# richhiey/YourMT3

Measured on AMD Instinct MI355X. Metric: audio-sec transcribed / wall-sec (RTF), higher is better.
Workload: dtype bf16; 1 GPU; BASELINE configs[1]: MT3 base (T5-small dims, 6+6 layers, d512, 8x64 heads, d_ff 2048, vocab 1536), 2.048 s / 16 kHz / 128-mel segments (256 encoder frames), greedy decode forced to 1024 tokens, seeded random weights; segments_per_gpu=64, global_batch=64, decode_len=1024, frames=256, parallelism=dp1 (segments sharded, token ids all-gathered over RCCL)

## Files before the change

yourmt3_amd/csrc/dec_chain.hip:

```cpp
#include <cstdlib>

#include "common.h"
#include "kernels.h"

namespace {

#include "dec_chain_body.h"

template <int MODE3, bool W2F>
__global__ __launch_bounds__(512) void dec_chain_kernel(const bf16_t* __restrict__ pW0, const bf16_t* __restrict__ pW1, const bf16_t* __restrict__ pW2,
                                                        const bf16_t* __restrict__ pW3, const bf16_t* __restrict__ pAttn, float* pH, int row0, int R,
                                                        ChainArgs c) {
    extern __shared__ __attribute__((aligned(16))) char smem[];
    chain_stages<MODE3, W2F>(pW0, pW1, pW2, pW3, pAttn, pH, row0, R, c, smem, blockIdx.x);
}

__global__ void chain_poison_kernel(const unsigned* sync, int32_t* tokens, float* scores, long long n) {
    if (sync[CHAIN_ABORT_WORD] == 0u) return;
    for (long long i = (long long)blockIdx.x * blockDim.x + threadIdx.x; i < n; i += (long long)gridDim.x * blockDim.x) {
        tokens[i] = INT32_MIN;
        if (scores) scores[i] = __builtin_nanf("");
    }
}

constexpr size_t CHAIN_LDS = (size_t)(8 * 16 * 16 + 16) * 4 + (size_t)8 * 2 * 16 * (2048 / 8 * 2 + 16);
constexpr size_t CHAIN_LDS_W2F = (size_t)(8 * 16 * 16 + 16) * 4 + (size_t)8 * 16 * (2048 / 8 * 2 + 16);
constexpr size_t CHAIN_LDS_NORM = (size_t)(8 * 16 * 32 + 16) * 4 + (size_t)8 * 3 * 16 * (512 / 8 * 2 + 16);
static_assert(CHAIN_LDS >= CHAIN_LDS_NORM && CHAIN_LDS_W2F >= CHAIN_LDS_NORM, "NORM stage LDS");
static_assert(CHAIN_LDS_W2F <= 80 * 1024, "two workgroups per CU");

}

int init_chain_kernels() {
    int rc = 0;
    rc |= hipFuncSetAttribute(reinterpret_cast<const void*>(dec_chain_kernel<DG_NORM_QKV_CACHE, false>), hipFuncAttributeMaxDynamicSharedMemorySize, (int)CHAIN_LDS) != hipSuccess;
    rc |= hipFuncSetAttribute(reinterpret_cast<const void*>(dec_chain_kernel<DG_NORM_LOGITS, false>), hipFuncAttributeMaxDynamicSharedMemorySize, (int)CHAIN_LDS) != hipSuccess;
    rc |= hipFuncSetAttribute(reinterpret_cast<const void*>(dec_chain_kernel<DG_NORM_QKV_CACHE, true>), hipFuncAttributeMaxDynamicSharedMemorySize, (int)CHAIN_LDS_W2F) != hipSuccess;
    rc |= hipFuncSetAttribute(reinterpret_cast<const void*>(dec_chain_kernel<DG_NORM_LOGITS, true>), hipFuncAttributeMaxDynamicSharedMemorySize, (int)CHAIN_LDS_W2F) != hipSuccess;
    return rc ? -2 : 0;
}

static bool chain_w2f() {
    static const bool v = [] { const char* e = getenv("YMT3_CHAIN_W2F"); return e && e[0] == '1'; }();
    return v;
}

bool dec_chain_fits(int n_cus) {
    int a = 0, b = 0;
    if (chain_w2f()) {
        if (hipOccupancyMaxActiveBlocksPerMultiprocessor(&a, dec_chain_kernel<DG_NORM_QKV_CACHE, true>, 512, CHAIN_LDS_W2F) != hipSuccess) return false;
        if (hipOccupancyMaxActiveBlocksPerMultiprocessor(&b, dec_chain_kernel<DG_NORM_LOGITS, true>, 512, CHAIN_LDS_W2F) != hipSuccess) return false;
    } else {
        if (hipOccupancyMaxActiveBlocksPerMultiprocessor(&a, dec_chain_kernel<DG_NORM_QKV_CACHE, false>, 512, CHAIN_LDS) != hipSuccess) return false;
        if (hipOccupancyMaxActiveBlocksPerMultiprocessor(&b, dec_chain_kernel<DG_NORM_LOGITS, false>, 512, CHAIN_LDS) != hipSuccess) return false;
    }
    return (long long)(a < b ? a : b) * n_cus >= 256;
}

int launch_dec_chain(const ChainArgs& c, hipStream_t stream) {
    if (c.R <= 0) return 0;
    if (c.R > 16 * CHAIN_TILES_MAX || c.d_ff != 2048 || c.N3 % 32 || c.N3 / 32 < 32 || c.N3 / 32 > 64 || !c.sync || (c.mode3 != DG_NORM_QKV_CACHE && c.mode3 != DG_NORM_LOGITS))
        return -1;
    const int n_mt = (c.R + 15) / 16;
    const int grid = n_mt <= 4 ? 256 : 64 * n_mt;
    if (chain_w2f()) {
        if (c.mode3 == DG_NORM_QKV_CACHE)
            dec_chain_kernel<DG_NORM_QKV_CACHE, true><<<grid, 512, CHAIN_LDS_W2F, stream>>>(c.w0, c.w1, c.w2, c.w3, c.attn, c.h, c.row0, c.R, c);
        else
            dec_chain_kernel<DG_NORM_LOGITS, true><<<grid, 512, CHAIN_LDS_W2F, stream>>>(c.w0, c.w1, c.w2, c.w3, c.attn, c.h, c.row0, c.R, c);
    } else if (c.mode3 == DG_NORM_QKV_CACHE)
        dec_chain_kernel<DG_NORM_QKV_CACHE, false><<<grid, 512, CHAIN_LDS, stream>>>(c.w0, c.w1, c.w2, c.w3, c.attn, c.h, c.row0, c.R, c);
    else
        dec_chain_kernel<DG_NORM_LOGITS, false><<<grid, 512, CHAIN_LDS, stream>>>(c.w0, c.w1, c.w2, c.w3, c.attn, c.h, c.row0, c.R, c);
    return 0;
}

int launch_chain_poison(const unsigned* sync, int32_t* tokens, float* scores, long long n, hipStream_t stream) {
    if (!sync || !tokens || n <= 0) return 0;
    chain_poison_kernel<<<64, 256, 0, stream>>>(sync, tokens, scores, n);
    return 0;
}
```

yourmt3_amd/csrc/dec_chain_body.h:

```cpp
#pragma once

#ifndef YMT3_TID
#define YMT3_TID threadIdx.x
#endif
#ifndef YMT3_POLL_PAUSE
#define YMT3_POLL_PAUSE do { } while (0)
#endif

typedef unsigned u32x4 __attribute__((ext_vector_type(4)));
constexpr int DKV = 64;
constexpr int AGENT = 16;
constexpr unsigned long long SPIN_LIMIT = 100000000ull;

#define CH_STAMP_IN(c) do { if ((c).stamp && YMT3_TID == 0) (c).stamp[2 * blockIdx.x] = wall_clock64(); } while (0)
#define CH_MARK(c, k) do { if ((c).stamp && YMT3_TID == 0) (c).stamp[512 + 8 * blockIdx.x + (k)] = wall_clock64(); } while (0)
#define CH_STAMP_OUT(c) do { if ((c).stamp && (YMT3_TID & 63) == 0) atomicMax((c).stamp + 2 * blockIdx.x + 1, (unsigned long long)wall_clock64()); } while (0)

__device__ __forceinline__ __amdgpu_buffer_rsrc_t raw_rsrc(const void* p) {
    return __builtin_amdgcn_make_buffer_rsrc(const_cast<void*>(p), 0, 0x7fffffff, 0x00020000);
}
__device__ __forceinline__ u32x4 ld16_agent(__amdgpu_buffer_rsrc_t r, int byte_off) { return __builtin_amdgcn_raw_buffer_load_b128(r, byte_off, 0, AGENT); }
__device__ __forceinline__ float ld_agent(const float* p) { return __hip_atomic_load(p, __ATOMIC_RELAXED, __HIP_MEMORY_SCOPE_AGENT); }
__device__ __forceinline__ void st_agent(float* p, float v) { __hip_atomic_store(p, v, __ATOMIC_RELAXED, __HIP_MEMORY_SCOPE_AGENT); }
__device__ __forceinline__ void st_agent(uint32_t* p, uint32_t v) { __hip_atomic_store(p, v, __ATOMIC_RELAXED, __HIP_MEMORY_SCOPE_AGENT); }
__device__ __forceinline__ void st2_agent(float* p, float2 v) {
    __hip_atomic_store(reinterpret_cast<unsigned long long*>(p), __builtin_bit_cast(unsigned long long, v), __ATOMIC_RELAXED, __HIP_MEMORY_SCOPE_AGENT);
}

template <int K, int NT>
struct Geo {
    static constexpr int KW = K / 8, KS = KW / 32, COLS = 16 * NT, PITCH = KW * 2 + 16, STRIP = 16 * PITCH;
    static constexpr int LPRW = KW * 2 / 16, RPIW = 64 / LPRW, NIA = 16 / RPIW, NIW = NIA * NT;
    static constexpr int LPRX = KW * 4 / 16, RPIX = 64 / LPRX, NIX = 16 / RPIX;
};

template <int K, int NT>
__device__ __forceinline__ void load_w(const bf16_t* W, int n0, u32x4 (&wv)[Geo<K, NT>::NIW]) {
    using G = Geo<K, NT>;
    const int lane = YMT3_TID & 63, wave = YMT3_TID >> 6;
#pragma unroll
    for (int i = 0; i < G::NIW; ++i)
        wv[i] = *reinterpret_cast<const u32x4*>(W + (size_t)(n0 + i * G::RPIW + lane / G::LPRW) * K + wave * G::KW + (lane % G::LPRW) * 8);
}

template <int K>
__device__ __forceinline__ void load_w_frag(const bf16_t* W, int n0, u32x4 (&wf)[Geo<K, 1>::KS]) {
    using G = Geo<K, 1>;
    const int lane = YMT3_TID & 63, wave = YMT3_TID >> 6, li = lane & 15, g = lane >> 4;
#pragma unroll
    for (int ks = 0; ks < G::KS; ++ks)
        wf[ks] = *reinterpret_cast<const u32x4*>(W + (size_t)(n0 + li) * K + wave * G::KW + ks * 32 + g * 8);
}

__device__ __forceinline__ unsigned* chain_counter(unsigned* sync, int boundary, int mt, int replica) {
    return sync + ((boundary * CHAIN_TILES_MAX + mt) * 8 + replica) * CHAIN_LINE;
}
__device__ __forceinline__ void chain_wait(unsigned* sync, int boundary, int mt, unsigned target, unsigned* host_abort, unsigned* abort_at = nullptr, int nsub = 1) {
    if (YMT3_TID < 64) {
        const int lane = YMT3_TID;
        const unsigned* cnt = chain_counter(sync, boundary, mt + 4 * (lane < nsub ? lane : 0), blockIdx.x & 7);
        const unsigned each = target / (unsigned)nsub;
        unsigned* abort_word = abort_at ? abort_at : sync + CHAIN_ABORT_WORD;
        unsigned long long t0 = 0;
        unsigned polls = 0;
        for (;;) {
            unsigned v = each;
            if (lane < nsub) v = __hip_atomic_load(cnt, __ATOMIC_RELAXED, __HIP_MEMORY_SCOPE_AGENT);
            if (__ballot(v < each) == 0ull) break;
            YMT3_POLL_PAUSE;
            if ((++polls & 63u) == 0u) {
                const unsigned long long now = wall_clock64();
                if (t0 == 0) t0 = now;
                if (__hip_atomic_load(abort_word, __ATOMIC_RELAXED, __HIP_MEMORY_SCOPE_AGENT) || now - t0 > SPIN_LIMIT) {
                    if (lane == 0) {
                        __hip_atomic_store(abort_word, 1u, __ATOMIC_RELAXED, __HIP_MEMORY_SCOPE_AGENT);
                        if (host_abort) __hip_atomic_store(host_abort, 1u, __ATOMIC_RELAXED, __HIP_MEMORY_SCOPE_SYSTEM);
                    }
                    break;
                }
            }
        }
    }
    __syncthreads();
}
__device__ __forceinline__ void counter_wait(const unsigned* cnt, unsigned target, unsigned* abort_word, unsigned* host_abort) {
    if (YMT3_TID == 0) {
        unsigned long long t0 = 0;
        unsigned polls = 0;
        while (__hip_atomic_load(cnt, __ATOMIC_RELAXED, __HIP_MEMORY_SCOPE_AGENT) < target) {
            YMT3_POLL_PAUSE;
            if ((++polls & 63u) == 0u) {
                const unsigned long long now = wall_clock64();
                if (t0 == 0) t0 = now;
                if (__hip_atomic_load(abort_word, __ATOMIC_RELAXED, __HIP_MEMORY_SCOPE_AGENT) || now - t0 > SPIN_LIMIT) {
                    __hip_atomic_store(abort_word, 1u, __ATOMIC_RELAXED, __HIP_MEMORY_SCOPE_AGENT);
                    if (host_abort) __hip_atomic_store(host_abort, 1u, __ATOMIC_RELAXED, __HIP_MEMORY_SCOPE_SYSTEM);
                    break;
                }
            }
        }
    }
    __syncthreads();
}
__device__ __forceinline__ void counter_signal(unsigned* cnt, int n, int stride) {
    asm volatile("s_waitcnt vmcnt(0)" ::: "memory");
    __syncthreads();
    if ((int)YMT3_TID < n) __hip_atomic_fetch_add(cnt + YMT3_TID * stride, 1u, __ATOMIC_RELAXED, __HIP_MEMORY_SCOPE_AGENT);
}
__device__ __forceinline__ void chain_signal(unsigned* sync, int boundary, int mt, int sub = 0) {
    asm volatile("s_waitcnt vmcnt(0)" ::: "memory");
    __syncthreads();
    if (YMT3_TID < 8) __hip_atomic_fetch_add(chain_counter(sync, boundary, mt + 4 * sub, YMT3_TID), 1u, __ATOMIC_RELAXED, __HIP_MEMORY_SCOPE_AGENT);
}

template <int K, int NT>
__device__ __forceinline__ float2 mfma_reduce(char* sA, char* sW, float* red) {
    using G = Geo<K, NT>;
    const int tid = YMT3_TID, lane = tid & 63, wave = tid >> 6, li = lane & 15, g = lane >> 4;
    f32x4 acc[NT];
#pragma unroll
    for (int c = 0; c < NT; ++c) acc[c] = (f32x4){0.f, 0.f, 0.f, 0.f};
#pragma unroll
    for (int ks = 0; ks < G::KS; ++ks) {
        const int off = li * G::PITCH + (ks * 32 + g * 8) * 2;
        const bf16x8 af = *reinterpret_cast<const bf16x8*>(sA + off);
#pragma unroll
        for (int c = 0; c < NT; ++c) {
            const bf16x8 wf = *reinterpret_cast<const bf16x8*>(sW + c * G::STRIP + off);
            acc[c] = __builtin_amdgcn_mfma_f32_16x16x32_bf16(wf, af, acc[c], 0, 0, 0);
        }
    }
#pragma unroll
    for (int c = 0; c < NT; ++c)
        *reinterpret_cast<float4*>(red + ((wave * 16 + li) * G::COLS + c * 16 + g * 4)) = make_float4(acc[c][0], acc[c][1], acc[c][2], acc[c][3]);
    __syncthreads();
    float2 s = make_float2(0.f, 0.f);
    if (tid < 16 * 8 * NT) {
        const int mr = tid / (8 * NT), nq = (tid % (8 * NT)) * 2;
        s = *reinterpret_cast<const float2*>(red + (mr * G::COLS + nq));
#pragma unroll
        for (int w = 1; w < 8; ++w) {
            const float2 t = *reinterpret_cast<const float2*>(red + ((w * 16 + mr) * G::COLS + nq));
            s.x += t.x; s.y += t.y;
        }
    }
    return s;
}

template <int K>
__device__ __forceinline__ float2 mfma_reduce_wfrag(char* sA, const u32x4 (&wfr)[Geo<K, 1>::KS], float* red) {
    using G = Geo<K, 1>;
    const int tid = YMT3_TID, lane = tid & 63, wave = tid >> 6, li = lane & 15, g = lane >> 4;
    f32x4 acc = (f32x4){0.f, 0.f, 0.f, 0.f};
#pragma unroll
    for (int ks = 0; ks < G::KS; ++ks) {
        const bf16x8 af = *reinterpret_cast<const bf16x8*>(sA + li * G::PITCH + (ks * 32 + g * 8) * 2);
        acc = __builtin_amdgcn_mfma_f32_16x16x32_bf16(__builtin_bit_cast(bf16x8, wfr[ks]), af, acc, 0, 0, 0);
    }
    *reinterpret_cast<float4*>(red + ((wave * 16 + li) * 16 + g * 4)) = make_float4(acc[0], acc[1], acc[2], acc[3]);
    __syncthreads();
    float2 s = make_float2(0.f, 0.f);
    if (tid < 16 * 8) {
        const int mr = tid / 8, nq = (tid % 8) * 2;
        s = *reinterpret_cast<const float2*>(red + (mr * 16 + nq));
#pragma unroll
        for (int w = 1; w < 8; ++w) {
            const float2 t = *reinterpret_cast<const float2*>(red + ((w * 16 + mr) * 16 + nq));
            s.x += t.x; s.y += t.y;
        }
    }
    return s;
}

__device__ __forceinline__ float2 resid_out(float2 hold, float2 s, float* pH, float* pSsq, int ssq_stride, int m, int n, int nt_idx, bool live) {
    float2 o = make_float2(0.f, 0.f);
    if (live) {
        o = make_float2(hold.x + s.x, hold.y + s.y);
        st2_agent(pH + (size_t)m * 512 + n, o);
    }
    float q = add_sep(mul_sep(o.x, o.x), mul_sep(o.y, o.y));
    q = sum8(q);
    if (live && (YMT3_TID & 7) == 0) st_agent(pSsq + (size_t)nt_idx * ssq_stride + m, q);
    return o;
}

__device__ __forceinline__ f32x4 norm_gain(const float* gain) {
    using G = Geo<512, 2>;
    return *reinterpret_cast<const f32x4*>(gain + (YMT3_TID >> 6) * G::KW + ((YMT3_TID & 63) % G::LPRX) * 4);
}
template <int NT>
__device__ __forceinline__ void norm_park(char* smem, u32x4 (&wv)[Geo<512, NT>::NIW]) {
    using G = Geo<512, NT>;
    const int lane = YMT3_TID & 63, wave = YMT3_TID >> 6;
    char* sW = smem + (8 * 16 * G::COLS + 16) * 4 + wave * (1 + NT) * G::STRIP + G::STRIP;
#pragma unroll
    for (int i = 0; i < G::NIW; ++i)
        *reinterpret_cast<u32x4*>(sW + (i * G::RPIW + lane / G::LPRW) * G::PITCH + (lane % G::LPRW) * 16) = wv[i];
}

template <int MODE, bool INL = false>
__device__ __forceinline__ void norm_tile(const ChainArgs& c, const float* pH, int row0, int R, const f32x4 gv, int N, int nt_idx, int mt_idx,
                                          int step, char* smem) {
    using G = Geo<512, 2>;
    constexpr int NT = 2;
    float* red = reinterpret_cast<float*>(smem);
    float* sscale = red + 8 * 16 * G::COLS;
    char* strips = smem + (8 * 16 * G::COLS + 16) * 4;
    const int tid = YMT3_TID, lane = tid & 63, wave = tid >> 6;
    const int n0 = nt_idx * G::COLS, m0 = row0 + mt_idx * 16, m_end = row0 + R;
    char* sA = strips + wave * (1 + NT) * G::STRIP;
    char* sW = sA + G::STRIP;
    const __amdgpu_buffer_rsrc_t rx = raw_rsrc(pH);
    f32x4 xv[G::NIX];
#pragma unroll
    for (int i = 0; i < G::NIX; ++i) {
        int mm = m0 + i * G::RPIX + lane / G::LPRX;
        mm = mm < m_end ? mm : m_end - 1;
        xv[i] = __builtin_bit_cast(f32x4, ld16_agent(rx, (mm * 512 + wave * G::KW + (lane % G::LPRX) * 4) * 4));
    }
    float ss = 0.f;
    if (tid < 16 * 8) {
        const int mm = m0 + (tid >> 3) < m_end ? m0 + (tid >> 3) : m_end - 1;
#pragma unroll
        for (int j = 0; j < 4; ++j) ss += ld_agent(c.ssq + (size_t)((tid & 7) * 4 + j) * c.ssq_stride + mm);
    }
    ss = sum8(ss);
    if (tid < 16 * 8 && (tid & 7) == 0) sscale[tid >> 3] = rsqrtf(ss / 512.f + c.eps);
    __syncthreads();
#pragma unroll
    for (int i = 0; i < G::NIX; ++i) {
        const int row = i * G::RPIX + lane / G::LPRX;
        const float sc = sscale[row];
        *reinterpret_cast<uint2*>(sA + row * G::PITCH + (lane % G::LPRX) * 8) =
            make_uint2(pack_bf16x2(xv[i][0] * sc * gv[0], xv[i][1] * sc * gv[1]), pack_bf16x2(xv[i][2] * sc * gv[2], xv[i][3] * sc * gv[3]));
    }
    float2 s = mfma_reduce<512, NT>(sA, sW, red);
    const bool epi = tid < 16 * 8 * NT;
    const int mr = tid / (8 * NT), nq = (tid % (8 * NT)) * 2;
    const int m = m0 + mr, n = n0 + nq;
    if (!(epi && m < m_end)) return;
    if constexpr (MODE == DG_NORM_LOGITS) {
        *reinterpret_cast<float2*>(c.logits + (size_t)m * N + n) = s;
    } else if constexpr (MODE == DG_NORM_BF16_RELU) {
        s.x = fmaxf(s.x, 0.f); s.y = fmaxf(s.y, 0.f);
        st_agent(reinterpret_cast<uint32_t*>(c.dff + (size_t)m * N + n), pack_bf16x2(s.x, s.y));
    } else {
        const uint32_t pk = pack_bf16x2(s.x, s.y);
        const int inner = c.H * DKV;
        if (n < inner) {
            if constexpr (INL) st_agent(reinterpret_cast<uint32_t*>(c.out_q + (size_t)m * inner + n), pk);
            else *reinterpret_cast<uint32_t*>(c.out_q + (size_t)m * inner + n) = pk;
        } else {
            const int nn = n - inner, kv = nn / inner, hh = (nn % inner) >> 6, dd = nn & 63;
            bf16_t* cache = kv ? c.vcache : c.kcache;
            if constexpr (INL) st_agent(reinterpret_cast<uint32_t*>(cache + (((size_t)m * c.H + hh) * c.L + step) * DKV + dd), pk);
            else *reinterpret_cast<uint32_t*>(cache + (((size_t)m * c.H + hh) * c.L + step) * DKV + dd) = pk;
        }
    }
}

struct ChainInLaunch {
    const unsigned* attn_done;
    unsigned attn_target;
    unsigned* qkv_done;
    unsigned long long* mark;
    int tiles_free;
};
template <int MODE3, bool W2F, bool INL = false>
__device__ __forceinline__ void chain_stages(const bf16_t* __restrict__ pW0, const bf16_t* __restrict__ pW1, const bf16_t* __restrict__ pW2,
                                             const bf16_t* __restrict__ pW3, const bf16_t* __restrict__ pAttn, float* pH, int row0, int R,
                                             const ChainArgs& c, char* smem, int t, const ChainInLaunch in = ChainInLaunch{}) {
    using G0 = Geo<512, 1>;
    using G1 = Geo<512, 2>;
    using G2 = Geo<2048, 1>;
    const int tid = YMT3_TID, lane = tid & 63, wave = tid >> 6;
    const int n_mt = (R + 15) / 16, m_end = row0 + R;
    const int nsub_all = c.nsub ? c.nsub : 0x444;
    const int nsub0 = n_mt <= 4 ? nsub_all & 15 : 1, nsub1 = n_mt <= 4 ? (nsub_all >> 4) & 15 : 1, nsub2 = n_mt <= 4 ? (nsub_all >> 8) & 15 : 1;
    const int mt = n_mt <= 4 ? (t >> 3) & 3 : t >> 6, nt = n_mt <= 4 ? (t >> 5) * 8 + (t & 7) : t & 63;
    const int n_nt3 = c.N3 / 32;
    const bool has0 = mt < n_mt && nt < 32, has1 = mt < n_mt, has3 = mt < n_mt && nt < n_nt3;
    const int nt0 = nt & 31, mt0 = mt, nt1 = nt, mt1 = mt, nt3 = nt < n_nt3 ? nt : nt - n_nt3, mt3 = mt;

    u32x4 w0[G0::NIW], av[G0::NIA];
    load_w<512, 1>(pW0, nt0 * 16, w0);
    const int m0 = row0 + mt0 * 16;
    const bool epi0 = tid < 16 * 8;
    const int mr0 = tid / 8, nq0 = (tid % 8) * 2;
    const int mE = m0 + mr0, nE = nt0 * 16 + nq0;
    const bool live0 = has0 && epi0 && mE < m_end;
    float2 hold = make_float2(0.f, 0.f);
    float2 hp[8];
    if constexpr (!INL) {
#pragma unroll
        for (int i = 0; i < G0::NIA; ++i) {
            int mm = m0 + i * G0::RPIW + lane / G0::LPRW;
            mm = mm < m_end ? mm : m_end - 1;
            av[i] = *reinterpret_cast<const u32x4*>(pAttn + (size_t)mm * 512 + wave * G0::KW + (lane % G0::LPRW) * 8);
        }
        if (live0) hold = *reinterpret_cast<const float2*>(pH + (size_t)mE * 512 + nE);
        if (c.part && live0) {
#pragma unroll
            for (int w = 0; w < 8; ++w) hp[w] = *reinterpret_cast<const float2*>(c.part + ((size_t)mE * 8 + w) * 512 + nE);
        }
    }
    int step = 0;
    if constexpr (MODE3 == DG_NORM_QKV_CACHE) {
        const int mq = row0 + mt3 * 16 + tid / 16;
        step = c.row_pos ? c.row_pos[mq < m_end ? mq : m_end - 1] : c.shared->step;
    }
    if constexpr (INL) {
        if (mt < n_mt) counter_wait(in.attn_done, in.attn_target, c.sync_abort, c.host_abort);
        if (in.mark && YMT3_TID == 0) in.mark[0] = wall_clock64();
        if (has0) {
            const __amdgpu_buffer_rsrc_t rat = raw_rsrc(pAttn);
#pragma unroll
            for (int i = 0; i < G0::NIA; ++i) {
                int mm = m0 + i * G0::RPIW + lane / G0::LPRW;
                mm = mm < m_end ? mm : m_end - 1;
                av[i] = ld16_agent(rat, (mm * 512 + wave * G0::KW + (lane % G0::LPRW) * 8) * 2);
            }
            if (live0) {
                hold = __builtin_bit_cast(float2, __hip_atomic_load(reinterpret_cast<const unsigned long long*>(pH + (size_t)mE * 512 + nE), __ATOMIC_RELAXED, __HIP_MEMORY_SCOPE_AGENT));
#pragma unroll
                for (int w = 0; w < 8; ++w)
                    hp[w] = __builtin_bit_cast(float2, __hip_atomic_load(reinterpret_cast<const unsigned long long*>(c.part + ((size_t)mE * 8 + w) * 512 + nE),
                                                                          __ATOMIC_RELAXED, __HIP_MEMORY_SCOPE_AGENT));
            }
        }
    }
    __builtin_amdgcn_sched_barrier(0);
    u32x4 w1[G1::NIW], w2[W2F ? G2::KS : G2::NIW], w3[G1::NIW];
    load_w<512, 2>(pW1, nt1 * 32, w1);
    const f32x4 g1 = norm_gain(c.gain1);
    __builtin_amdgcn_sched_barrier(0);
    CH_STAMP_IN(c);

    float2 o0 = make_float2(0.f, 0.f);
    if (has0) {
        float* red = reinterpret_cast<float*>(smem);
        char* strips = smem + (8 * 16 * 16 + 16) * 4;
        char* sA = strips + wave * 2 * G0::STRIP;
        char* sW = sA + G0::STRIP;
#pragma unroll
        for (int i = 0; i < G0::NIW; ++i) {
            const int off = (i * G0::RPIW + lane / G0::LPRW) * G0::PITCH + (lane % G0::LPRW) * 16;
            *reinterpret_cast<u32x4*>(sW + off) = w0[i];
            *reinterpret_cast<u32x4*>(sA + off) = av[i];
        }
        const float2 s = mfma_reduce<512, 1>(sA, sW, red);
        if (c.part && live0) {
            float2 sp = hp[0];
#pragma unroll
            for (int w = 1; w < 8; ++w) { sp.x += hp[w].x; sp.y += hp[w].y; }
            hold.x += sp.x; hold.y += sp.y;
        }
        o0 = resid_out(hold, s, pH, c.ssq, c.ssq_stride, mE, nE, nt0, live0);
        CH_MARK(c, 0);
        chain_signal(c.sync, 0, mt0, nt0 & (nsub0 - 1));
        CH_MARK(c, 1);
    }
    if constexpr (W2F) load_w_frag<2048>(pW2, nt0 * 16, w2);
    else load_w<2048, 1>(pW2, nt0 * 16, w2);
    __builtin_amdgcn_sched_barrier(0);
    if (has1) {
        norm_park<2>(smem, w1);
        chain_wait(c.sync, 0, mt1, 32u, c.host_abort, c.sync_abort, nsub0);
        CH_MARK(c, 2);
        norm_tile<DG_NORM_BF16_RELU>(c, pH, row0, R, g1, c.d_ff, nt1, mt1, 0, smem);
        CH_MARK(c, 3);
        chain_signal(c.sync, 1, mt1, nt1 & (nsub1 - 1));
        CH_MARK(c, 4);
    }
    load_w<512, 2>(pW3, nt3 * 32, w3);
    const f32x4 g3 = norm_gain(c.gain3);
    __builtin_amdgcn_sched_barrier(0);
    if (has0) {
        float* red = reinterpret_cast<float*>(smem);
        char* strips = smem + (8 * 16 * 16 + 16) * 4;
        char* sA = strips + wave * (W2F ? 1 : 2) * G2::STRIP;
        if constexpr (!W2F) {
            char* sW = sA + G2::STRIP;
#pragma unroll
            for (int i = 0; i < G2::NIW; ++i)
                *reinterpret_cast<u32x4*>(sW + (i * G2::RPIW + lane / G2::LPRW) * G2::PITCH + (lane % G2::LPRW) * 16) = w2[i];
        }
        chain_wait(c.sync, 1, mt0, (unsigned)(c.d_ff / 32), c.host_abort, c.sync_abort, nsub1);
        CH_MARK(c, 5);
        const __amdgpu_buffer_rsrc_t ra = raw_rsrc(c.dff);
        u32x4 dv[G2::NIA];
#pragma unroll
        for (int i = 0; i < G2::NIA; ++i) {
            int mm = m0 + i * G2::RPIW + lane / G2::LPRW;
            mm = mm < m_end ? mm : m_end - 1;
            dv[i] = ld16_agent(ra, (mm * 2048 + wave * G2::KW + (lane % G2::LPRW) * 8) * 2);
        }
#pragma unroll
        for (int i = 0; i < G2::NIA; ++i)
            *reinterpret_cast<u32x4*>(sA + (i * G2::RPIW + lane / G2::LPRW) * G2::PITCH + (lane % G2::LPRW) * 16) = dv[i];
        float2 s;
        if constexpr (W2F) s = mfma_reduce_wfrag<2048>(sA, w2, red);
        else s = mfma_reduce<2048, 1>(sA, sA + G2::STRIP, red);
        resid_out(o0, s, pH, c.ssq, c.ssq_stride, mE, nE, nt0, live0);
        CH_MARK(c, 6);
        chain_signal(c.sync, 2, mt0, nt0 & (nsub2 - 1));
    }
    if (has3) {
        norm_park<2>(smem, w3);
        chain_wait(c.sync, 2, mt3, 32u, c.host_abort, c.sync_abort, nsub2);
        CH_MARK(c, 7);
        norm_tile<MODE3, INL>(c, pH, row0, R, g3, c.N3, nt3, mt3, step, smem);
    }
    if constexpr (INL && MODE3 == DG_NORM_QKV_CACHE) {
        if (mt < n_mt) {
            if (has3) counter_signal(in.qkv_done + (size_t)((in.tiles_free ? mt3 * 8 : 0) + ((nt3 & 15) >> 1)) * CHAIN_LINE, in.tiles_free ? 1 : 4, 8 * CHAIN_LINE);
        }
    }
    CH_STAMP_OUT(c);
}
```

Measured before the change: 574.1 audio_s/wall_s.

## Split chain GEMM row tiles into half tiles for small-batch launches

```diff
diff --git a/yourmt3_amd/csrc/dec_chain.hip b/yourmt3_amd/csrc/dec_chain.hip
--- a/yourmt3_amd/csrc/dec_chain.hip
+++ b/yourmt3_amd/csrc/dec_chain.hip
@@ -11,6 +11,13 @@
 __global__ __launch_bounds__(512) void dec_chain_kernel(const bf16_t* __restrict__ pW0, const bf16_t* __restrict__ pW1, const bf16_t* __restrict__ pW2,
                                                         const bf16_t* __restrict__ pW3, const bf16_t* __restrict__ pAttn, float* pH, int row0, int R,
                                                         ChainArgs c) {
+    extern __shared__ __attribute__((aligned(16))) char smem[];
+    chain_stages<MODE3, W2F, false, true>(pW0, pW1, pW2, pW3, pAttn, pH, row0, R, c, smem, blockIdx.x);
+}
+template <int MODE3, bool W2F>
+__global__ __launch_bounds__(512) void dec_chain_rows_kernel(const bf16_t* __restrict__ pW0, const bf16_t* __restrict__ pW1, const bf16_t* __restrict__ pW2,
+                                                             const bf16_t* __restrict__ pW3, const bf16_t* __restrict__ pAttn, float* pH, int row0, int R,
+                                                             ChainArgs c) {
     extern __shared__ __attribute__((aligned(16))) char smem[];
     chain_stages<MODE3, W2F>(pW0, pW1, pW2, pW3, pAttn, pH, row0, R, c, smem, blockIdx.x);
 }
@@ -29,14 +36,34 @@
 static_assert(CHAIN_LDS >= CHAIN_LDS_NORM && CHAIN_LDS_W2F >= CHAIN_LDS_NORM, "NORM stage LDS");
 static_assert(CHAIN_LDS_W2F <= 80 * 1024, "two workgroups per CU");
 
+template <int MODE3, bool W2F>
+int chain_set_lds(size_t lds) {
+    int rc = 0;
+    rc |= hipFuncSetAttribute(reinterpret_cast<const void*>(dec_chain_kernel<MODE3, W2F>), hipFuncAttributeMaxDynamicSharedMemorySize, (int)lds) != hipSuccess;
+    rc |= hipFuncSetAttribute(reinterpret_cast<const void*>(dec_chain_rows_kernel<MODE3, W2F>), hipFuncAttributeMaxDynamicSharedMemorySize, (int)lds) != hipSuccess;
+    return rc;
+}
+template <int MODE3, bool W2F>
+int chain_blocks_per_cu(size_t lds) {
+    int a = 0, b = 0;
+    if (hipOccupancyMaxActiveBlocksPerMultiprocessor(&a, dec_chain_kernel<MODE3, W2F>, 512, lds) != hipSuccess) return 0;
+    if (hipOccupancyMaxActiveBlocksPerMultiprocessor(&b, dec_chain_rows_kernel<MODE3, W2F>, 512, lds) != hipSuccess) return 0;
+    return a < b ? a : b;
+}
+template <int MODE3, bool W2F>
+void chain_launch(const ChainArgs& c, int n_mt, size_t lds, hipStream_t stream) {
+    if (n_mt <= 4) dec_chain_kernel<MODE3, W2F><<<256, 512, lds, stream>>>(c.w0, c.w1, c.w2, c.w3, c.attn, c.h, c.row0, c.R, c);
+    else dec_chain_rows_kernel<MODE3, W2F><<<64 * n_mt, 512, lds, stream>>>(c.w0, c.w1, c.w2, c.w3, c.attn, c.h, c.row0, c.R, c);
+}
+
 }
 
 int init_chain_kernels() {
     int rc = 0;
-    rc |= hipFuncSetAttribute(reinterpret_cast<const void*>(dec_chain_kernel<DG_NORM_QKV_CACHE, false>), hipFuncAttributeMaxDynamicSharedMemorySize, (int)CHAIN_LDS) != hipSuccess;
-    rc |= hipFuncSetAttribute(reinterpret_cast<const void*>(dec_chain_kernel<DG_NORM_LOGITS, false>), hipFuncAttributeMaxDynamicSharedMemorySize, (int)CHAIN_LDS) != hipSuccess;
-    rc |= hipFuncSetAttribute(reinterpret_cast<const void*>(dec_chain_kernel<DG_NORM_QKV_CACHE, true>), hipFuncAttributeMaxDynamicSharedMemorySize, (int)CHAIN_LDS_W2F) != hipSuccess;
-    rc |= hipFuncSetAttribute(reinterpret_cast<const void*>(dec_chain_kernel<DG_NORM_LOGITS, true>), hipFuncAttributeMaxDynamicSharedMemorySize, (int)CHAIN_LDS_W2F) != hipSuccess;
+    rc |= chain_set_lds<DG_NORM_QKV_CACHE, false>(CHAIN_LDS);
+    rc |= chain_set_lds<DG_NORM_LOGITS, false>(CHAIN_LDS);
+    rc |= chain_set_lds<DG_NORM_QKV_CACHE, true>(CHAIN_LDS_W2F);
+    rc |= chain_set_lds<DG_NORM_LOGITS, true>(CHAIN_LDS_W2F);
     return rc ? -2 : 0;
 }
 
@@ -46,13 +73,13 @@
 }
 
 bool dec_chain_fits(int n_cus) {
-    int a = 0, b = 0;
+    int a, b;
     if (chain_w2f()) {
-        if (hipOccupancyMaxActiveBlocksPerMultiprocessor(&a, dec_chain_kernel<DG_NORM_QKV_CACHE, true>, 512, CHAIN_LDS_W2F) != hipSuccess) return false;
-        if (hipOccupancyMaxActiveBlocksPerMultiprocessor(&b, dec_chain_kernel<DG_NORM_LOGITS, true>, 512, CHAIN_LDS_W2F) != hipSuccess) return false;
+        a = chain_blocks_per_cu<DG_NORM_QKV_CACHE, true>(CHAIN_LDS_W2F);
+        b = chain_blocks_per_cu<DG_NORM_LOGITS, true>(CHAIN_LDS_W2F);
     } else {
-        if (hipOccupancyMaxActiveBlocksPerMultiprocessor(&a, dec_chain_kernel<DG_NORM_QKV_CACHE, false>, 512, CHAIN_LDS) != hipSuccess) return false;
-        if (hipOccupancyMaxActiveBlocksPerMultiprocessor(&b, dec_chain_kernel<DG_NORM_LOGITS, false>, 512, CHAIN_LDS) != hipSuccess) return false;
+        a = chain_blocks_per_cu<DG_NORM_QKV_CACHE, false>(CHAIN_LDS);
+        b = chain_blocks_per_cu<DG_NORM_LOGITS, false>(CHAIN_LDS);
     }
     return (long long)(a < b ? a : b) * n_cus >= 256;
 }
@@ -62,16 +89,13 @@
     if (c.R > 16 * CHAIN_TILES_MAX || c.d_ff != 2048 || c.N3 % 32 || c.N3 / 32 < 32 || c.N3 / 32 > 64 || !c.sync || (c.mode3 != DG_NORM_QKV_CACHE && c.mode3 != DG_NORM_LOGITS))
         return -1;
     const int n_mt = (c.R + 15) / 16;
-    const int grid = n_mt <= 4 ? 256 : 64 * n_mt;
     if (chain_w2f()) {
-        if (c.mode3 == DG_NORM_QKV_CACHE)
-            dec_chain_kernel<DG_NORM_QKV_CACHE, true><<<grid, 512, CHAIN_LDS_W2F, stream>>>(c.w0, c.w1, c.w2, c.w3, c.attn, c.h, c.row0, c.R, c);
-        else
-            dec_chain_kernel<DG_NORM_LOGITS, true><<<grid, 512, CHAIN_LDS_W2F, stream>>>(c.w0, c.w1, c.w2, c.w3, c.attn, c.h, c.row0, c.R, c);
+        if (c.mode3 == DG_NORM_QKV_CACHE) chain_launch<DG_NORM_QKV_CACHE, true>(c, n_mt, CHAIN_LDS_W2F, stream);
+        else chain_launch<DG_NORM_LOGITS, true>(c, n_mt, CHAIN_LDS_W2F, stream);
     } else if (c.mode3 == DG_NORM_QKV_CACHE)
-        dec_chain_kernel<DG_NORM_QKV_CACHE, false><<<grid, 512, CHAIN_LDS, stream>>>(c.w0, c.w1, c.w2, c.w3, c.attn, c.h, c.row0, c.R, c);
+        chain_launch<DG_NORM_QKV_CACHE, false>(c, n_mt, CHAIN_LDS, stream);
     else
-        dec_chain_kernel<DG_NORM_LOGITS, false><<<grid, 512, CHAIN_LDS, stream>>>(c.w0, c.w1, c.w2, c.w3, c.attn, c.h, c.row0, c.R, c);
+        chain_launch<DG_NORM_LOGITS, false>(c, n_mt, CHAIN_LDS, stream);
     return 0;
 }
 
diff --git a/yourmt3_amd/csrc/dec_chain_body.h b/yourmt3_amd/csrc/dec_chain_body.h
--- a/yourmt3_amd/csrc/dec_chain_body.h
+++ b/yourmt3_amd/csrc/dec_chain_body.h
@@ -266,35 +266,41 @@
     unsigned long long* mark;
     int tiles_free;
 };
-template <int MODE3, bool W2F, bool INL = false>
+template <int MODE3, bool W2F, bool INL = false, bool HALF = false>
 __device__ __forceinline__ void chain_stages(const bf16_t* __restrict__ pW0, const bf16_t* __restrict__ pW1, const bf16_t* __restrict__ pW2,
                                              const bf16_t* __restrict__ pW3, const bf16_t* __restrict__ pAttn, float* pH, int row0, int R,
                                              const ChainArgs& c, char* smem, int t, const ChainInLaunch in = ChainInLaunch{}) {
     using G0 = Geo<512, 1>;
     using G1 = Geo<512, 2>;
     using G2 = Geo<2048, 1>;
+    static_assert(!(HALF && INL), "half-row tiles: the launch form only");
+    static_assert(G0::RPIW == 8 && G0::NIA == 2 && G2::RPIW * (G2::NIA / 2) == 8, "a half tile is whole load instructions");
+    constexpr int NIA0 = HALF ? G0::NIA / 2 : G0::NIA, NIA2 = HALF ? G2::NIA / 2 : G2::NIA;
     const int tid = YMT3_TID, lane = tid & 63, wave = tid >> 6;
     const int n_mt = (R + 15) / 16, m_end = row0 + R;
+    const bool merged = HALF || n_mt <= 4;
     const int nsub_all = c.nsub ? c.nsub : 0x444;
-    const int nsub0 = n_mt <= 4 ? nsub_all & 15 : 1, nsub1 = n_mt <= 4 ? (nsub_all >> 4) & 15 : 1, nsub2 = n_mt <= 4 ? (nsub_all >> 8) & 15 : 1;
-    const int mt = n_mt <= 4 ? (t >> 3) & 3 : t >> 6, nt = n_mt <= 4 ? (t >> 5) * 8 + (t & 7) : t & 63;
+    const int nsub0 = merged ? nsub_all & 15 : 1, nsub1 = merged ? (nsub_all >> 4) & 15 : 1, nsub2 = merged ? (nsub_all >> 8) & 15 : 1;
+    constexpr unsigned target02 = HALF ? 64u : 32u;
+    const int mt = merged ? (t >> 3) & 3 : t >> 6, nt = merged ? (t >> 5) * 8 + (t & 7) : t & 63;
     const int n_nt3 = c.N3 / 32;
-    const bool has0 = mt < n_mt && nt < 32, has1 = mt < n_mt, has3 = mt < n_mt && nt < n_nt3;
+    const bool has0 = mt < n_mt && (HALF || nt < 32), has1 = mt < n_mt, has3 = mt < n_mt && nt < n_nt3;
     const int nt0 = nt & 31, mt0 = mt, nt1 = nt, mt1 = mt, nt3 = nt < n_nt3 ? nt : nt - n_nt3, mt3 = mt;
-
-    u32x4 w0[G0::NIW], av[G0::NIA];
+    const int r0 = HALF ? (nt >> 5) * 8 : 0, z0 = 8 - r0;
+
+    u32x4 w0[G0::NIW], av[NIA0];
     load_w<512, 1>(pW0, nt0 * 16, w0);
     const int m0 = row0 + mt0 * 16;
     const bool epi0 = tid < 16 * 8;
     const int mr0 = tid / 8, nq0 = (tid % 8) * 2;
     const int mE = m0 + mr0, nE = nt0 * 16 + nq0;
-    const bool live0 = has0 && epi0 && mE < m_end;
+    const bool live0 = has0 && epi0 && mE < m_end && (!HALF || (mr0 & 8) == r0);
     float2 hold = make_float2(0.f, 0.f);
     float2 hp[8];
     if constexpr (!INL) {
 #pragma unroll
-        for (int i = 0; i < G0::NIA; ++i) {
-            int mm = m0 + i * G0::RPIW + lane / G0::LPRW;
+        for (int i = 0; i < NIA0; ++i) {
+            int mm = m0 + r0 + i * G0::RPIW + lane / G0::LPRW;
             mm = mm < m_end ? mm : m_end - 1;
             av[i] = *reinterpret_cast<const u32x4*>(pAttn + (size_t)mm * 512 + wave * G0::KW + (lane % G0::LPRW) * 8);
         }
@@ -346,7 +352,8 @@
         for (int i = 0; i < G0::NIW; ++i) {
             const int off = (i * G0::RPIW + lane / G0::LPRW) * G0::PITCH + (lane % G0::LPRW) * 16;
             *reinterpret_cast<u32x4*>(sW + off) = w0[i];
-            *reinterpret_cast<u32x4*>(sA + off) = av[i];
+            if constexpr (HALF) *reinterpret_cast<u32x4*>(sA + off) = i * G0::RPIW == r0 ? av[0] : (u32x4){0u, 0u, 0u, 0u};
+            else *reinterpret_cast<u32x4*>(sA + off) = av[i];
         }
         const float2 s = mfma_reduce<512, 1>(sA, sW, red);
         if (c.part && live0) {
@@ -365,7 +372,7 @@
     __builtin_amdgcn_sched_barrier(0);
     if (has1) {
         norm_park<2>(smem, w1);
-        chain_wait(c.sync, 0, mt1, 32u, c.host_abort, c.sync_abort, nsub0);
+        chain_wait(c.sync, 0, mt1, target02, c.host_abort, c.sync_abort, nsub0);
         CH_MARK(c, 2);
         norm_tile<DG_NORM_BF16_RELU>(c, pH, row0, R, g1, c.d_ff, nt1, mt1, 0, smem);
         CH_MARK(c, 3);
@@ -385,29 +392,39 @@
             for (int i = 0; i < G2::NIW; ++i)
                 *reinterpret_cast<u32x4*>(sW + (i * G2::RPIW + lane / G2::LPRW) * G2::PITCH + (lane % G2::LPRW) * 16) = w2[i];
         }
+        if constexpr (HALF) {
+#pragma unroll
+            for (int i = 0; i < NIA2; ++i)
+                *reinterpret_cast<u32x4*>(sA + z0 * G2::PITCH + (i * G2::RPIW + lane / G2::LPRW) * G2::PITCH + (lane % G2::LPRW) * 16) = (u32x4){0u, 0u, 0u, 0u};
+        }
         chain_wait(c.sync, 1, mt0, (unsigned)(c.d_ff / 32), c.host_abort, c.sync_abort, nsub1);
         CH_MARK(c, 5);
         const __amdgpu_buffer_rsrc_t ra = raw_rsrc(c.dff);
-        u32x4 dv[G2::NIA];
-#pragma unroll
-        for (int i = 0; i < G2::NIA; ++i) {
-            int mm = m0 + i * G2::RPIW + lane / G2::LPRW;
+        u32x4 dv[NIA2];
+#pragma unroll
+        for (int i = 0; i < NIA2; ++i) {
+            int mm = m0 + r0 + i * G2::RPIW + lane / G2::LPRW;
             mm = mm < m_end ? mm : m_end - 1;
             dv[i] = ld16_agent(ra, (mm * 2048 + wave * G2::KW + (lane % G2::LPRW) * 8) * 2);
         }
 #pragma unroll
-        for (int i = 0; i < G2::NIA; ++i)
-            *reinterpret_cast<u32x4*>(sA + (i * G2::RPIW + lane / G2::LPRW) * G2::PITCH + (lane % G2::LPRW) * 16) = dv[i];
+        for (int i = 0; i < NIA2; ++i)
+            *reinterpret_cast<u32x4*>(sA + r0 * G2::PITCH + (i * G2::RPIW + lane / G2::LPRW) * G2::PITCH + (lane % G2::LPRW) * 16) = dv[i];
+#ifdef YMT3_MARK_S2_OPERANDS
+        CH_MARK(c, 6);
+#endif
         float2 s;
         if constexpr (W2F) s = mfma_reduce_wfrag<2048>(sA, w2, red);
         else s = mfma_reduce<2048, 1>(sA, sA + G2::STRIP, red);
         resid_out(o0, s, pH, c.ssq, c.ssq_stride, mE, nE, nt0, live0);
+#ifndef YMT3_MARK_S2_OPERANDS
         CH_MARK(c, 6);
+#endif
         chain_signal(c.sync, 2, mt0, nt0 & (nsub2 - 1));
     }
     if (has3) {
         norm_park<2>(smem, w3);
-        chain_wait(c.sync, 2, mt3, 32u, c.host_abort, c.sync_abort, nsub2);
+        chain_wait(c.sync, 2, mt3, target02, c.host_abort, c.sync_abort, nsub2);
         CH_MARK(c, 7);
         norm_tile<MODE3, INL>(c, pH, row0, R, g3, c.N3, nt3, mt3, step, smem);
     }
```

Measured after the change: 573.8 audio_s/wall_s, median of 3. About the same (-0.1%).
